# ParthaEth/GIF

Measured on AMD Instinct MI355X. Metric: G+D train-step images/sec at 256x256, batch 32/GPU, higher is better.
Workload: dtype f32

## Files before the change

### gif_amd/_lib.py

```python
import ctypes
import os

import torch

_HERE = os.path.dirname(os.path.abspath(__file__))
LIB_PATH = os.path.join(_HERE, "libgif_hip.so")

c_int, c_i64, c_float, c_void_p = ctypes.c_int, ctypes.c_int64, ctypes.c_float, ctypes.c_void_p


def knob(name, default):
    if os.environ.get("GIF_EXPERIMENTAL", "0") in ("", "0"):
        return default
    return os.environ.get(name, default)
P = c_void_p


class ConvGeom(ctypes.Structure):
    _fields_ = [(n, ctypes.c_int32) for n in ("B", "Hb", "Wb", "Cb", "Hs", "Ws", "Cs", "KH", "KW", "stride", "pad")]


class ConvEpilogue(ctypes.Structure):
    _fields_ = [("in_scale", P), ("out_scale", P), ("bias", P), ("residual", P),
                ("act", ctypes.c_int32), ("slope", c_float), ("gain", c_float),
# ... 90 lines not shown
    "gif_conv3x3_winograd_wgrad_f32": (c_int, [P, P, P, P, P, P, P, c_int, c_int, c_int, c_int, c_int, c_int, P]),
    "gif_conv3x3_winograd_wgrad_f32x3": (c_int, [P, P, P, P, P, P, P, c_int, c_int, c_int, c_int, c_int, c_int, P]),
    "gif_conv3x3_winograd_wgrad_f32h2": (c_int, [P, P, P, P, P, P, P, c_int, c_int, c_int, c_int, c_int, c_int, P]),
    "gif_winograd_unpack_wgrad_f32": (c_int, [P, P, c_int, c_int, c_int, c_int, c_int, c_i64, c_i64, c_i64, c_i64, c_float, P]),
    "gif_texture_pair_loss_partials": (c_int, [c_i64]),
    "gif_texture_pair_loss_f32": (c_int, [P, P, P, P, P, P, P, c_int, c_i64, P]),
    "gif_texture_pair_loss_bwd_f32": (c_int, [P, P, P, P, P, P, P, c_int, c_i64, P]),
    "gif_resize_f32": (c_int, [P, P, c_i64, c_int, c_int, c_int, c_int, c_int, P]),
    "gif_resize_bwd_f32": (c_int, [P, P, c_i64, c_int, c_int, c_int, c_int, c_int, P]),
    "gif_upfirdn2d_f32": (c_int, [P, P, P] + [c_int] * 13 + [EP, P]),
    "gif_bias_act_f32": (c_int, [P, P, P, P, c_i64, c_int, c_float, c_float, P]),
    "gif_colsum_partial_floats": (c_i64, [c_i64, c_int]),
    "gif_bias_act_bwd_f32": (c_int, [P, P, P, P, P, c_i64, c_int, c_float, c_float, P]),
    "gif_colsum_f32": (c_int, [P, P, P, c_i64, c_int, P]),
    "gif_mul_reduce_chunks": (c_int, [c_i64]),
    "gif_mul_reduce_f32": (c_int, [P, P, P, P, P, P, c_int, c_i64, c_int, P]),
    "gif_pack_nhwc_f32": (c_int, [P, c_int, c_int, ctypes.POINTER(c_i64), P, c_int, c_int, ctypes.POINTER(c_i64), P, c_int, c_int, c_int, c_int, P]),
    "gif_pack_nhwc_f16": (c_int, [P, c_int, c_int, ctypes.POINTER(c_i64), P, c_int, c_int, ctypes.POINTER(c_i64), P, c_int, c_int, c_int, c_int, P]),
    "gif_unpack_nhwc_f32": (c_int, [P, P, c_int, c_int, c_int, c_int, c_int, c_int, P]),
    "gif_unpack_nhwc_f16": (c_int, [P, P, c_int, c_int, c_int, c_int, c_int, c_int, P]),
    "gif_bilinear_down_f32": (c_int, [P, P, c_int, c_int, c_int, c_int, c_int, P]),
    "gif_act_inv_mul_reduce_f32": (c_int, [P, P, P, P, P, P, c_int, c_i64, c_int, c_float, c_float, P]),
    "gif_mbstd_fwd_f32": (c_int, [P, P, P, c_int, c_int, c_int, c_int, c_int, c_int, P]),
    "gif_mbstd_bwd_f32": (c_int, [P, P, P, c_int, c_int, c_int, c_int, c_int, c_int, P]),
    "gif_sqnorm_per_sample_f32": (c_int, [P, P, c_int, c_i64, P]),
    "gif_conv2d_pack_dims_f16": (c_int, [c_int, c_int, ctypes.POINTER(c_int), ctypes.POINTER(c_int)]),
    "gif_pack_weight_f16": (c_int, [P, P, c_int, c_int, c_int, c_int, c_int, c_int, c_i64, c_i64, c_i64, c_i64, c_float, P]),
    "gif_conv2d_f16_halo_eligible": (c_int, [c_int] * 7),
    "gif_conv2d_f16_halo_enable": (c_int, [c_int]),
    "gif_conv2d_fwd_f16": (c_int, [P, P, P, GP, EP, P]),
    "gif_conv2d_bwd_data_f16": (c_int, [P, P, P, GP, EP, P]),
    "gif_conv2d_wgrad_dims_f16": (c_int, [c_int, c_int, ctypes.POINTER(c_int), ctypes.POINTER(c_int)]),
    "gif_conv2d_wgrad_splits_f16": (c_int, [GP]),
    "gif_conv2d_wgrad_f16": (c_int, [P, P, P, P, P, GP, c_int, P]),
    "gif_upfirdn2d_f16": (c_int, [P, P, P] + [c_int] * 13 + [EP, P]),
    "gif_bias_act_f16": (c_int, [P, P, P, P, c_i64, c_int, c_float, c_float, P]),
    "gif_bias_act_bwd_f16": (c_int, [P, P, P, P, P, c_i64, c_int, c_float, c_float, P]),
    "gif_colsum_f16": (c_int, [P, P, P, c_i64, c_int, P]),
    "gif_mul_reduce_f16": (c_int, [P, P, P, P, P, P, c_int, c_i64, c_int, P]),
    "gif_act_inv_mul_reduce_f16": (c_int, [P, P, P, P, P, P, c_int, c_i64, c_int, c_float, c_float, P]),
    "gif_linear_nt_f32": (c_int, [P, P, P, P] + [c_int] * 7 + [c_float, c_int, c_float, c_float, P]),
    "gif_linear_nn_f32": (c_int, [P, P, P] + [c_int] * 7 + [c_float, P]),
    "gif_linear_tn_f32": (c_int, [P, P, P] + [c_int] * 6 + [c_float, P]),
    "gif_linear_bank_fwd_f32": (c_int, [P, c_int, c_int, c_int, ctypes.POINTER(LinearBankSeg), c_int, c_float, P]),
    "gif_linear_bank_bwd_f32": (c_int, [P, c_int, c_int, c_int, ctypes.POINTER(LinearBankSeg), c_int, c_float, P, c_int, c_int, P]),
    "gif_weight_sq_sum_f32": (c_int, [P, P, c_int, c_int, c_int, P]),
    "gif_style_demod_f32": (c_int, [P, P, P] + [c_int] * 7 + [c_float, c_float, P]),
    "gif_style_demod_bwd_s_f32": (c_int, [P] * 6 + [c_int] * 7 + [c_float, P]),
    "gif_style_demod_bwd_w_f32": (c_int, [P] * 4 + [c_int] * 5 + [c_float, P]),
    "gif_demod_wgrad_f32": (c_int, [P, P, P, c_int, c_int, c_int, P]),
    "gif_adam_chunk_floats": (c_int, []),
    "gif_adam_ema_step_f32": (c_int, [P, c_int, P, P, P, c_float, c_float, c_float, c_float, ctypes.c_double, ctypes.c_double,
                                      c_float, c_int, P, P, P, P]),
    "gif_prof_enable": (c_int, [c_int]),
    "gif_prof_read": (c_int, [c_int, ctypes.POINTER(ctypes.c_double), ctypes.POINTER(ctypes.c_double), ctypes.POINTER(c_i64)]),
}

_lib = None


class GifHipError(RuntimeError):
    pass


def load():
    global _lib
    if _lib is not None:
        return _lib
    if not os.path.exists(LIB_PATH):
        raise GifHipError(
            f"{LIB_PATH} not found: the HIP extension is not built. Run `make -C gif_amd/csrc` "
            "(or __graft_entry__.build()). gif_amd has no fallback path.")
    lib = ctypes.CDLL(LIB_PATH)
    for name, (res, args) in PROTOTYPES.items():
        fn = getattr(lib, name)
        fn.restype, fn.argtypes = res, args
    _lib = lib
    return lib


def check(rc, what):
    if rc != 0:
        msg = load().gif_last_error().decode(errors="replace")
        raise GifHipError(f"{what} failed (rc={rc}): {msg}")


def marshal(entry, args):
    out = list(args)
    for i, a in enumerate(out):
        if isinstance(a, torch.Tensor):
            if not a.is_contiguous():
                raise GifHipError(f"{entry}: argument {i} is not contiguous (shape {list(a.shape)}, strides {list(a.stride())})")
            out[i] = a.data_ptr()
    return out


def launch(entry, device, *args):
    fn, argv = getattr(load(), entry), marshal(entry, args)
    if device.index in (None, torch.cuda.current_device()):
        return check(fn(*argv, torch.cuda.current_stream().cuda_stream), entry)
    with torch.cuda.device(device):
        check(fn(*argv, torch.cuda.current_stream().cuda_stream), entry)


def workspace(nbytes, device):
    return torch.empty((max(nbytes // 4, 1),), device=device, dtype=torch.float32)
# ... 13 lines not shown
```

### gif_amd/functional.py

```python
import weakref

import torch
from torch.autograd import Function

from . import ops
from .ops import ConvSpec


class ActPort:
    __slots__ = ("alias", "slope", "gain", "want_bias", "parts", "y_ref")

    def __init__(self, slope, gain, want_bias):
        self.alias, self.slope, self.gain, self.want_bias = None, float(slope), float(gain), bool(want_bias)
        self.parts = []
        self.y_ref = None

    def cfg(self):
        return (self.slope, self.gain, self.want_bias, self.parts, self.y_ref)


def _observed(t):
    return t.retains_grad or bool(t._backward_hooks)


def _port_live(cfg):
    if cfg is None:
        return False
    y = cfg[4]() if cfg[4] is not None else None
    return y is None or not _observed(y)


def _file_part(parts, part):
    if not parts:
        torch.autograd.Variable._execution_engine.queue_callback(parts.clear)
    parts.append(part)


def _take_port(x, identity=False):
    port = getattr(x, "_gif_port", None)
    if (port is None or not ops.FUSE_GRAD or not torch.is_grad_enabled() or port.alias is None or not port.alias.requires_grad
            or (port.slope == 1.0 and port.gain == 1.0) != identity or _observed(x)):
        return None, None
    return port.alias, port.cfg()


_inputs_only = False


class inputs_only_backward:
    def __enter__(self):
        global _inputs_only
        self._prev, _inputs_only = _inputs_only, True

    def __exit__(self, *exc):
        global _inputs_only
        _inputs_only = self._prev
# ... 112 lines not shown
        return gs, gb, None, None, None, None, None


class ConvBiasActFn(Function):

    @staticmethod
    def forward(ctx, x, w, bias, spec, wscale, slope, gain, passthrough=False, in_port=None, parts=None, x_port=None):
        ctx.set_materialize_grads(False)
        ctx.pmask = _param_mask(x, w, bias)
        x = ops.nhwc(x)
        y, v = ops.conv_fwd(x, w, spec, wscale, keep_v=True, bias=bias, act=True, slope=slope, gain=gain)
        ctx.v = v if ctx.needs_input_grad[1] else None
        ctx.cfg = (spec, wscale, slope, gain, bias is not None)
        ctx.in_port, ctx.parts = in_port, parts
        ctx.save_for_backward(x, w, y)
        return y, y.detach(), (x.view_as(x) if passthrough else None)

    @staticmethod
    def backward(ctx, gy, g_port=None, g_alias=None):
        x, w, y = ctx.saved_tensors
        spec, ws, slope, gain, has_bias = ctx.cfg
        want_b = has_bias and _need(ctx, 2)
        gx = gw = None
        port = _port_on(ctx)
        gpre, gb = _producer_gpre(gy, g_port, y, want_b, slope, gain, ctx.parts)
        if gpre is not None:
            if ctx.needs_input_grad[0]:
                gx = _conv_dgrad(gpre, w, spec, tuple(x.shape[2:]), ws, g_alias, ctx.in_port if port else None, x)
            if _need(ctx, 1):
                gw = WgradFn.apply(gpre, x, spec, w.shape[0], w.shape[1], ws, ctx.v)
        elif ctx.needs_input_grad[0] and g_alias is not None:
            gx = _mask_into_port(ctx.in_port, g_alias, x) if port else g_alias
        return (None if port else gx), gw, (gb if want_b else None), None, None, None, None, None, None, None, (gx if port else None)


def _conv_dgrad(gpre, w, spec, big_hw, ws, residual, in_port, x):
    if in_port is None:
        return Conv2dFn.apply(gpre, w, spec, True, big_hw, ws, residual)
    slope, gain, want_b, parts = in_port[:4]
    fuse = ops.GradFuse(mask_src=x, mask_slope=slope, mask_gain=gain, want_colsum=want_b)
    gx = ops.conv_bwd_data(gpre, w, spec, big_hw, ws, residual=None if residual is None else ops.nhwc(residual), fuse=fuse)
    if want_b:
        _file_part(parts, fuse.colsum)
    return gx


def conv2d_bias_act(x, w, bias, stride=1, pad=0, wscale=1.0, slope=0.2, gain=2 ** 0.5, passthrough=False):
    x_port, in_port = _take_port(x)
    port = _new_port(True, slope, gain, bias)
    y, alias, x_alias = ConvBiasActFn.apply(x, w, bias, ConvSpec(w.shape[2], w.shape[3], stride, pad), wscale, slope, gain,
                                            bool(passthrough), in_port, None if port is None else port.parts, x_port)
    _tag(y, alias, port)
    return (y, x_alias) if passthrough else y


def conv2d(x, w, stride=1, pad=0, wscale=1.0, residual=None):
    return Conv2dFn.apply(x, w, ConvSpec(w.shape[2], w.shape[3], stride, pad), False, None, wscale, residual)


def conv_transpose2d(x, w, stride, pad, out_hw, wscale=1.0):
    return Conv2dFn.apply(x, w, ConvSpec(w.shape[2], w.shape[3], stride, pad), True, tuple(out_hw), wscale, None)


class LinearNtFn(Function):

    @staticmethod
    def forward(ctx, a, b, scale, n_pad):
        ctx.scale = scale
        ctx.pmask = _param_mask(a, b)
        ctx.save_for_backward(a, b)
        return ops.linear_nt(a, b, None, scale, n_pad=n_pad)

    @staticmethod
    def backward(ctx, g):
        a, b = ctx.saved_tensors
        N, K = b.shape
        ga = LinearNnFn.apply(g, b, ctx.scale, a.shape[1]) if _need(ctx, 0) else None
        gb = LinearTnFn.apply(g, a, ctx.scale, N, K) if _need(ctx, 1) else None
        return ga, gb, None, None


class LinearNnFn(Function):

    @staticmethod
    def forward(ctx, a, b, scale, k_pad):
        ctx.scale = scale
        ctx.pmask = _param_mask(a, b)
        ctx.save_for_backward(a, b)
        return ops.linear_nn(a, b, scale, k_pad=k_pad)

    @staticmethod
    def backward(ctx, g):
        a, b = ctx.saved_tensors
        N, K = b.shape
        ga = LinearNtFn.apply(g, b, ctx.scale, a.shape[1]) if _need(ctx, 0) else None
        gb = LinearTnFn.apply(a, g, ctx.scale, N, K) if _need(ctx, 1) else None
        return ga, gb, None, None


class LinearTnFn(Function):

    @staticmethod
    def forward(ctx, a, b, scale, N, K):
        ctx.scale = scale
        ctx.pmask = _param_mask(a, b)
        ctx.save_for_backward(a, b)
# ... 558 lines not shown
```

### gif_amd/layers.py

```python
import math
import os

import torch
from torch import nn
from torch.nn import functional as F

from . import _lib
from . import functional as GF
from .ops import cpad, pad4


_SKINNY_MAX_ROWS = int(_lib.knob("GIF_SKINNY_MAX_ROWS", "512"))


def _pad_vec(v, n):
    v = v.reshape(-1)
    k = n - v.numel()
    if k == 0:
        return v
    key = (v.device, v.dtype, k)
    tail = _ZERO_TAILS.get(key)
    if tail is None:
        tail = _ZERO_TAILS[key] = torch.zeros(k, device=v.device, dtype=v.dtype)
    return torch.cat([v, tail])
# ... 212 lines not shown
    def _padded_scales(self, style, in_act, dtype=torch.float32):
        return self.scales(style, in_act, cpad(self.out_channel, dtype))

    def forward_fused_act(self, input, style, residual, bias, slope=0.2, gain=2 ** 0.5):
        batch, in_act, height, width = input.shape
        s, d = self._padded_scales(style, in_act, input.dtype)
        w = self.weight.squeeze(0)
        if self.upsample:
            out = GF.modulated_conv2d(input, w.transpose(0, 1), s, d, stride=2, pad=0, transposed=True,
                                      out_hw=(2 * height + self.kernel_size - 2, 2 * width + self.kernel_size - 2),
                                      wscale=self.scale)
            return GF.blur_bias_act(out, self.blur.kernel, self.blur.pad, residual, bias, slope, gain)
        if self.downsample or d is None:
            return GF.bias_act(self.forward(input, style, scales=(s, d)), bias, residual, slope, gain)
        return GF.modulated_conv2d_act(input, w, s, d, residual, bias, self.padding, self.scale, slope, gain)

    def forward(self, input, style, scales=None):
        batch, in_act, height, width = input.shape
        s, d = self._padded_scales(style, in_act, input.dtype) if scales is None else scales
        w = self.weight.squeeze(0)
        if self.upsample:
            out = GF.modulated_conv2d(input, w.transpose(0, 1), s, d, stride=2, pad=0, transposed=True,
                                      out_hw=(2 * height + self.kernel_size - 2, 2 * width + self.kernel_size - 2),
                                      wscale=self.scale)
            out = self.blur(out)
        elif self.downsample:
            out = GF.modulated_conv2d(self.blur(input), w, s, d, stride=2, pad=0, wscale=self.scale)
        else:
            out = GF.modulated_conv2d(input, w, s, d, stride=1, pad=self.padding, wscale=self.scale, out_f32=self.out_fp32)
        return out


_STYLE_BANK = _lib.knob("GIF_STYLE_BANK", "1") != "0"


def modulation_bank(convs, style):
    if not _STYLE_BANK or len(convs) < 2:
        return
    x = style.reshape(-1, style.shape[-1])
    mods = [c.modulation for c in convs]
    m0 = mods[0]
    same = all(m.scale == m0.scale and m.lr_mul == 1 and m.bias is not None and m.activation is None and
               m.weight.shape[1] == m0.weight.shape[1] for m in mods)
    if not same or x.dtype != torch.float32 or x.shape[0] > _SKINNY_MAX_ROWS or any(c.in_channel > 1024 for c in convs):
        return
    weights = [m.weight for m in mods]
    if not GF.ops.linear_bank_ok(x, weights):
        return
    outs = GF.linear_bank(x, weights, [m.bias for m in mods], m0.scale)
    for c, o in zip(convs, outs):
        c._banked = (style, o)


class NoiseInjection(nn.Module):

    @staticmethod
    def small_init_weights(m):
        if hasattr(m, 'weight'):
            m.weight.data = torch.randn_like(m.weight) / 100
        if hasattr(m, 'bias'):
            m.bias.data.fill_(0.0001)

    def __init__(self, noise_in_chalnnels, noise_out_channels):
        super().__init__()
        self.noise_in_chalnnels = noise_in_chalnnels
        c = noise_in_chalnnels
        self.noise_conv = nn.Sequential(
            nn.Conv2d(c, 2 * c, 3, padding=1), nn.ReLU(),
            nn.Conv2d(2 * c, 4 * c, 3, padding=1), nn.ReLU(),
            nn.Conv2d(4 * c, noise_out_channels, 3, padding=1))
        self.noise_conv.apply(NoiseInjection.small_init_weights)

    def convolve(self, noise):
        h = noise
        for idx in (0, 2, 4):
            conv = self.noise_conv[idx]
            last = idx == 4
            h = GF.conv2d_bias_act(h, conv.weight, _pad_vec(conv.bias, cpad(conv.weight.shape[0], h.dtype)), 1, 1, 1.0,
                                   1.0 if last else 0.0, 1.0)
        return h

    def forward(self, image, noise):
        batch, _, height, width = image.shape
        if noise is None:
            noise = image.new_empty(batch, cpad(self.noise_in_chalnnels, image.dtype), height, width).normal_()
            noise[:, self.noise_in_chalnnels:] = 0
        return GF.bias_act(image, None, self.convolve(noise), 1.0, 1.0)


class ConstantInput(nn.Module):
    def __init__(self, channel, size=4):
        super().__init__()
        self.input = nn.Parameter(torch.randn(1, channel, size, size))

    def forward(self, input):
        return self.input.repeat(input.shape[0], 1, 1, 1)


class StyledConv(nn.Module):

    def __init__(self, in_channel, out_channel, kernel_size, noise_in_dims, style_dim=512, upsample=False,
                 blur_kernel=[1, 3, 3, 1], demodulate=True, apply_sqrt2_fac_in_eq_lin=False):
        super().__init__()
        self.conv = ModulatedConv2d(in_channel, out_channel, kernel_size, style_dim, upsample=upsample,
                                    blur_kernel=blur_kernel, demodulate=demodulate,
                                    apply_sqrt2_fac_in_eq_lin=apply_sqrt2_fac_in_eq_lin)
        self.noise = NoiseInjection(noise_in_dims, out_channel)
        self.activate = FusedLeakyReLU(out_channel)

    def forward(self, input, style, noise=None):
        if noise is None:
            return self.activate(self.noise(self.conv(input, style), noise=None))
        act = self.activate
        return self.conv.forward_fused_act(input, style, self.noise.convolve(noise),
                                           _pad_vec(act.bias, cpad(self.conv.out_channel, input.dtype)), act.negative_slope,
                                           act.scale)


class ToRGB(nn.Module):

    def __init__(self, in_channel, style_dim, upsample=True, blur_kernel=[1, 3, 3, 1],
                 apply_sqrt2_fac_in_eq_lin=False):
        super().__init__()
        if upsample:
            self.upsample = Upsample(blur_kernel)
        self.conv = ModulatedConv2d(in_channel, 3, 1, style_dim, demodulate=False,
                                    apply_sqrt2_fac_in_eq_lin=apply_sqrt2_fac_in_eq_lin)
        self.conv.out_fp32 = True
# ... 82 lines not shown
```

### gif_amd/ops.py

```python
import ctypes
import functools
import os
import weakref
from typing import NamedTuple, Optional

import torch

from . import _lib

CL = torch.channels_last


def _stream():
    return torch.cuda.current_stream().cuda_stream


def _device_guard(fn):
    @functools.wraps(fn)
    def wrapped(*args, **kw):
        dev = None
        for a in args + tuple(kw.values()):
            if isinstance(a, torch.Tensor) and a.is_cuda:
                if dev is None:
                    dev = a.device
# ... 549 lines not shown
    _lib.check(_fn("unpack_nhwc", g.dtype)(g.data_ptr(), out.data_ptr(), B, H, W, cp, c_off, C, _stream()), "unpack_nhwc")
    return out


def act_inv_mul_reduce(g, y, residual, bias, slope, gain):
    lib = _lib.load()
    g, y = nhwc(g), nhwc(y)
    _same_dtype(g, y, "act_inv_mul_reduce")
    B, C, H, W = y.shape
    if B * H * W == 0:
        return torch.zeros((B, C), device=y.device, dtype=torch.float32)
    nchunk = lib.gif_mul_reduce_chunks(H * W)
    out = torch.empty((B, C), device=y.device, dtype=torch.float32)
    partial = torch.empty((B * nchunk * C,), device=y.device, dtype=torch.float32)
    _lib.check(_fn("act_inv_mul_reduce", y.dtype)(g.data_ptr(), y.data_ptr(), _p(residual), _p(bias), out.data_ptr(),
                                                  partial.data_ptr(), B, H * W, C, slope, gain, _stream()),
               "act_inv_mul_reduce")
    return out


def mbstd_fwd(x, G, Cy):
    lib = _lib.load()
    x = nhwc(x)
    if x.dtype != torch.float32:
        raise _lib.GifHipError("minibatch stddev is fp32 only (functional.minibatch_stddev casts the 4x4 tensor)")
    B, C, H, W = x.shape
    y = empty_nhwc(B, Cy, H, W, x.device)
    stat = torch.empty((B // G,), device=x.device, dtype=torch.float32)
    _lib.check(lib.gif_mbstd_fwd_f32(x.data_ptr(), y.data_ptr(), stat.data_ptr(), B, H, W, C, Cy, G, _stream()), "mbstd_fwd")
    return y, stat


def mbstd_bwd(x, gy, G):
    lib = _lib.load()
    x, gy = nhwc(x), nhwc(gy)
    B, C, H, W = x.shape
    Cy = gy.shape[1]
    gx = empty_nhwc(B, C, H, W, x.device)
    _lib.check(lib.gif_mbstd_bwd_f32(x.data_ptr(), gy.data_ptr(), gx.data_ptr(), B, H, W, C, Cy, G, _stream()), "mbstd_bwd")
    return gx


def sqnorm_per_sample(g):
    lib = _lib.load()
    if not g.is_cuda or g.dtype != torch.float32:
        raise _lib.GifHipError("sqnorm_per_sample needs an fp32 device tensor")
    g = g if g.is_contiguous() or g.is_contiguous(memory_format=CL) else g.contiguous()
    B = g.shape[0]
    out = torch.empty((B,), device=g.device, dtype=torch.float32)
    _lib.check(lib.gif_sqnorm_per_sample_f32(g.data_ptr(), out.data_ptr(), B, g.numel() // max(B, 1), _stream()), "sqnorm")
    return out


_raster_ws = {}
_RASTER_WS_MAX = 8


def _raster_ws_drop(lib, key):
    ws = _raster_ws.pop(key, None)
    if ws is not None:
        lib.gif_rasterize_assume_clean_workspace(ws.data_ptr(), 0)


def _raster_workspace(lib, dev, B, F, h, w):
    key = (dev.index, torch.cuda.current_stream().cuda_stream, B, F, h, w)
    ws = _raster_ws.get(key)
    if ws is None:
        if len(_raster_ws) >= _RASTER_WS_MAX:
            _raster_ws_drop(lib, next(iter(_raster_ws)))
        ws = torch.zeros((max((lib.gif_rasterize_workspace_bytes(B, F, h, w) + 7) // 8, 1),), device=dev, dtype=torch.int64)
        _raster_ws[key] = ws
        _lib.check(lib.gif_rasterize_assume_clean_workspace(ws.data_ptr(), 1), "rasterize_assume_clean_workspace")
    return key, ws


def rasterize(face_vertices, depth, tri, out3, h, w, face_colors=None):
    lib = _lib.load()
    B, F = face_vertices.shape[:2]
    f64 = face_vertices.dtype == torch.float64
    key, ws = _raster_workspace(lib, face_vertices.device, B, F, h, w)
    plain, colors = (lib.gif_rasterize_f64, lib.gif_rasterize_colors_f64) if f64 else (lib.gif_rasterize_f32,
                                                                                        lib.gif_rasterize_colors_f32)
    if face_colors is None:
        rc = plain(face_vertices.data_ptr(), depth.data_ptr(), tri.data_ptr(), out3.data_ptr(), B, F, h, w, ws.data_ptr(),
                   _stream())
    else:
        rc = colors(face_vertices.data_ptr(), face_colors.data_ptr(), depth.data_ptr(), tri.data_ptr(), out3.data_ptr(), B, F,
                    h, w, ws.data_ptr(), _stream())
    if rc != 0:
        _raster_ws_drop(lib, key)
    _lib.check(rc, "rasterize")


def _mask_u8(m, hw):
    if m is None:
        return None
    m = m.reshape(-1)
    if m.numel() != hw:
        raise _lib.GifHipError(f"texture_pair_loss: visibility mask has {m.numel()} elements, expected {hw}")
    return (m != 0).to(torch.uint8).contiguous()


def texture_pair_loss(a, b, ma, mb, f, gloss=None):
    lib = _lib.load()
    if not (a.is_cuda and b.is_cuda and f.is_cuda) or a.dtype != torch.float32 or a.dim() != 3 or a.shape != b.shape:
        raise _lib.GifHipError("texture_pair_loss: need two fp32 device textures [C,H,W] of the same shape (no CPU fallback)")
    a, b = a.contiguous(), b.contiguous()
    C, H, W = a.shape
    HW = H * W
    f = f.to(torch.float32).reshape(-1).contiguous()
    if f.numel() != HW:
        raise _lib.GifHipError(f"texture_pair_loss: face mask has {f.numel()} elements, expected {HW}")
    ma, mb = _mask_u8(ma, HW), _mask_u8(mb, HW)
    if gloss is None:
        partial = torch.empty((lib.gif_texture_pair_loss_partials(C * HW),), device=a.device, dtype=torch.float32)
        loss = torch.empty((), device=a.device, dtype=torch.float32)
        _lib.check(lib.gif_texture_pair_loss_f32(a.data_ptr(), b.data_ptr(), _p(ma), _p(mb), f.data_ptr(), partial.data_ptr(),
                                                 loss.data_ptr(), C, HW, _stream()), "texture_pair_loss")
        return loss
    ga = torch.empty_like(a)
    gloss = gloss.to(torch.float32).contiguous()
    _lib.check(lib.gif_texture_pair_loss_bwd_f32(a.data_ptr(), b.data_ptr(), _p(ma), _p(mb), f.data_ptr(), gloss.data_ptr(),
                                                 ga.data_ptr(), C, HW, _stream()), "texture_pair_loss_bwd")
    return ga


def resize(x, out_hw, mode: str, backward_to=None):
    lib = _lib.load()
    if not x.is_cuda or x.dtype != torch.float32 or x.dim() != 4:
        raise _lib.GifHipError("resize: need a 4-D fp32 device tensor (no CPU fallback)")
    if mode not in ("bilinear", "bicubic"):
        raise _lib.GifHipError(f"resize: mode {mode!r} not supported (bilinear | bicubic)")
    x = x.contiguous()
    B, C, H, W = x.shape
    m = 0 if mode == "bilinear" else 1
    if backward_to is None:
        Ho, Wo = out_hw
        y = torch.empty((B, C, Ho, Wo), device=x.device, dtype=torch.float32)
        _lib.check(lib.gif_resize_f32(x.data_ptr(), y.data_ptr(), B * C, H, W, Ho, Wo, m, _stream()), "resize")
        return y
    Hi, Wi = backward_to
    gx = torch.empty((B, C, Hi, Wi), device=x.device, dtype=torch.float32)
    _lib.check(lib.gif_resize_bwd_f32(x.data_ptr(), gx.data_ptr(), B * C, Hi, Wi, H, W, m, _stream()), "resize_bwd")
    return gx


for _name in ("pack_weight", "conv3x3_winograd", "conv_fwd", "conv_bwd_data", "conv3x3_winograd_wgrad", "conv_wgrad", "upfirdn2d",
              "bias_act", "bias_act_bwd", "colsum", "mul_reduce", "bilinear_down", "act_inv_mul_reduce", "mbstd_fwd", "mbstd_bwd",
              "sqnorm_per_sample", "rasterize", "texture_pair_loss", "resize"):
    globals()[_name] = _device_guard(globals()[_name])
del _name


def _mat(t, what):
    if not t.is_cuda or t.dtype != torch.float32 or t.dim() != 2:
        raise _lib.GifHipError(f"{what}: need a 2-D fp32 device tensor (no CPU fallback), got {tuple(t.shape)} {t.dtype} on {t.device}")
    return t if t.stride(1) == 1 and t.stride(0) >= t.shape[1] and t.data_ptr() % 16 == 0 and t.stride(0) % 4 == 0 else t.contiguous()


def linear_nt(a, b, bias=None, scale=1.0, act=False, slope=0.2, gain=1.0, n_pad=None):
    lib = _lib.load()
    a, b = _mat(a, "linear_nt"), _mat(b, "linear_nt")
    M = a.shape[0]
    N, K = b.shape
    assert a.shape[1] >= K, (a.shape, b.shape)
    n_pad = N if n_pad is None else n_pad
    c = torch.empty((M, n_pad), device=a.device, dtype=torch.float32)
    _lib.check(lib.gif_linear_nt_f32(a.data_ptr(), b.data_ptr(), _p(bias), c.data_ptr(), M, N, K, a.stride(0), b.stride(0), n_pad,
                                     n_pad, float(scale), 1 if act else 0, float(slope), float(gain), _stream()), "linear_nt")
    return c


LINEAR_BANK_MAX = 40


def linear_bank_ok(x, weights):
    K = weights[0].shape[1]
    return (0 < len(weights) <= LINEAR_BANK_MAX and x.dtype == torch.float32 and x.dim() == 2 and x.shape[1] >= K and K % 4 == 0
            and all(w.dim() == 2 and w.shape[1] == K and w.shape[0] % 8 == 0 and w.dtype == torch.float32 for w in weights))


def _bank_segs(weights):
    segs = (_lib.LinearBankSeg * len(weights))()
    keep = []
    for g, w in zip(segs, weights):
        w = _mat(w, "linear_bank")
        assert w.stride(0) == w.shape[1], "linear_bank: weight rows must be contiguous"
        keep.append(w)
        g.w, g.n = w.data_ptr(), w.shape[0]
    return segs, keep


def linear_bank_fwd(x, weights, biases, scale):
    lib = _lib.load()
    x = _mat(x, "linear_bank_fwd")
    M, K = x.shape[0], weights[0].shape[1]
    segs, keep = _bank_segs(weights)
    outs = []
    for g, w, b in zip(segs, weights, biases):
        o = torch.empty((M, w.shape[0]), device=x.device, dtype=torch.float32)
        if b is not None:
            assert b.dtype == torch.float32 and b.numel() == w.shape[0] and b.is_contiguous()
# ... 169 lines not shown
```

### include/gif_hip.h

```cpp
#ifndef GIF_HIP_H
#define GIF_HIP_H

#include <stdint.h>

#ifdef __cplusplus
extern "C" {
#endif

#define GIF_EINVAL (-1)
#define GIF_ENOSUP (-2)

typedef void* gif_stream_t;

const char* gif_last_error(void);
int gif_abi_version(void);

int gif_f16_overflow_clear(gif_stream_t stream);
int gif_f16_overflow_or_into(float* found_inf, gif_stream_t stream);
int gif_f16_overflow_watch(int on);

#define GIF_FP32_MFMA_NATIVE 0
#define GIF_FP32_MFMA_BF16X3 1
#define GIF_FP32_MFMA_F16X2 2
int gif_set_fp32_mfma_mode(int mode);
// ... 252 lines not shown
int gif_conv2d_bwd_data_f16(const void* small, const void* wp, void* big, const gif_conv_geom* g,
                            const gif_conv_epilogue* e, gif_stream_t stream);
int gif_conv2d_wgrad_dims_f16(int Cs, int Cb, int* RP, int* CP);
int gif_conv2d_wgrad_splits_f16(const gif_conv_geom* g);
int gif_conv2d_wgrad_f16(const void* small, const void* big, float* ws, const float* small_scale, const float* big_scale,
                         const gif_conv_geom* g, int nsplit, gif_stream_t stream);
int gif_upfirdn2d_f16(const void* x, const float* k, void* y, int B, int Hi, int Wi, int C, int Ho, int Wo, int up, int down,
                      int padx0, int pady0, int KH, int KW, int flip, const gif_conv_epilogue* e, gif_stream_t stream);
int gif_bias_act_f16(const void* x, const float* bias, const void* residual, void* y, int64_t npix, int C, float slope,
                     float gain, gif_stream_t stream);
int gif_bias_act_bwd_f16(const void* gy, const void* y, void* gx, float* gbias, float* partial, int64_t npix, int C,
                         float slope, float gain, gif_stream_t stream);
int gif_colsum_f16(const void* x, float* out, float* partial, int64_t npix, int C, gif_stream_t stream);
int gif_mul_reduce_f16(const void* a, const void* b, const float* scale, void* scaled, float* out, float* partial, int B,
                       int64_t HW, int C, gif_stream_t stream);
int gif_act_inv_mul_reduce_f16(const void* g, const void* y, const void* residual, const float* bias, float* out,
                               float* partial, int B, int64_t HW, int C, float slope, float gain, gif_stream_t stream);

int gif_linear_nt_f32(const float* A, const float* B, const float* bias, float* C, int M, int N, int K, int lda, int ldb,
                      int ldc, int cpad, float scale, int act, float slope, float gain, gif_stream_t stream);
int gif_linear_nn_f32(const float* A, const float* B, float* C, int M, int N, int K, int lda, int ldb, int ldc, int cpad,
                      float scale, gif_stream_t stream);
int gif_linear_tn_f32(const float* A, const float* B, float* C, int M, int N, int K, int lda, int ldb, int ldc, float scale,
                      gif_stream_t stream);

typedef struct gif_linear_bank_seg {
    const float* w;
    const float* bias;
    float* s;
    const float* gs;
    float* gw;
    float* gbias;
    int n;
    int reserved;
} gif_linear_bank_seg;
int gif_linear_bank_fwd_f32(const float* x, int M, int K, int ldx, const gif_linear_bank_seg* segs, int nseg, float scale,
                            gif_stream_t stream);
int gif_linear_bank_bwd_f32(const float* x, int M, int K, int ldx, const gif_linear_bank_seg* segs, int nseg, float scale, float* gx,
                            int ldgx, int gx_pad, gif_stream_t stream);

typedef struct gif_adam_chunk {
    float* param;
    float* ema;
    int64_t flat_offset;
    int32_t n;
    int32_t step_offset;
} gif_adam_chunk;
int gif_adam_chunk_floats(void);
int gif_adam_ema_step_f32(const gif_adam_chunk* chunks, int nchunks, const float* grad_flat, float* exp_avg_flat,
                          float* exp_avg_sq_flat, float lr, float beta1, float beta2, float eps, double bias_correction1,
                          double bias_correction2, float ema_decay, int has_ema, const float* inv_grad_scale,
                          const float* found_inf, const float* dev_step, gif_stream_t stream);

#ifdef __cplusplus
}
#endif
#endif
```

Before: 183.7.

## Fuse first two noise-injection convs into one tiled HIP kernel with fused backward

Adds a dedicated HIP kernel that runs the first two 3x3 convs of the NoiseInjection head (6->12->24 channels, ReLU) per spatial tile. The intermediate activation stays in LDS and the convs use fp32 MFMA. A matching backward kernel fuses the ReLU masks, the data gradient through conv2 and the per-tile bias-gradient partials, then reduces them in a second small kernel. The goal is to avoid separate launches and a global-memory round trip for the small-channel intermediate, which the generic conv path handles poorly. The trade-offs are a kernel specialised to fixed channel counts, extra recompute on tile halos, and an h1 tensor still written out when gradients are needed.

```diff
diff --git a/gif_amd/_lib.py b/gif_amd/_lib.py
--- a/gif_amd/_lib.py
+++ b/gif_amd/_lib.py
@@ -166,6 +166,9 @@
     "gif_adam_chunk_floats": (c_int, []),
     "gif_adam_ema_step_f32": (c_int, [P, c_int, P, P, P, c_float, c_float, c_float, c_float, ctypes.c_double, ctypes.c_double,
                                       c_float, c_int, P, P, P, P]),
+    "gif_noise_head_partial_floats": (c_i64, [c_int, c_int, c_int]),
+    "gif_noise_head_fwd_f32": (c_int, [P] * 7 + [c_int] * 3 + [c_i64] * 8 + [c_int, P]),
+    "gif_noise_head_bwd_data_f32": (c_int, [P] * 9 + [c_int] * 3 + [c_i64] * 4 + [c_int, P]),
     "gif_prof_enable": (c_int, [c_int]),
     "gif_prof_read": (c_int, [c_int, ctypes.POINTER(ctypes.c_double), ctypes.POINTER(ctypes.c_double), ctypes.POINTER(c_i64)]),
 }
diff --git a/gif_amd/csrc/noise_head.hip b/gif_amd/csrc/noise_head.hip
--- /dev/null
+++ b/gif_amd/csrc/noise_head.hip
@@ -0,0 +1,316 @@
+#include "common.h"
+
+namespace {
+
+typedef float f32x16 __attribute__((ext_vector_type(16)));
+using gif::f32x4_t;
+
+constexpr int TH = 16, TW = 32;
+constexpr int XH = TH + 4, XW = TW + 4;
+constexpr int HH = TH + 2, HW = TW + 2;
+constexpr int C0 = 6, C0S = 8, C1 = 12, C2 = 24;
+constexpr int NT = 256;
+constexpr int K1 = C0 * 9, K1_STEPS = (K1 + 3) / 4;
+constexpr int NPOS = HH * HW, NPOS_BLOCKS = (NPOS + 15) / 16;
+constexpr int kGridCap = 512;
+constexpr int kPartialC = C2 + C1;
+
+struct WStrides {
+    long o, i, y, x;
+};
+
+struct TileGrid {
+    int tiles_y, tiles_x;
+    long ntiles;
+};
+
+__device__ __forceinline__ void tile_origin(long tile, const TileGrid& tg, int& b, int& y0, int& x0) {
+    const long per_img = (long)tg.tiles_y * tg.tiles_x;
+    b = (int)(tile / per_img);
+    const int r = (int)(tile - (long)b * per_img);
+    y0 = (r / tg.tiles_x) * TH;
+    x0 = (r % tg.tiles_x) * TW;
+}
+
+__device__ __forceinline__ float relu(float v) { return v > 0.f ? v : 0.f; }
+
+template <bool kWantH1>
+__global__ __launch_bounds__(NT, 2) void noise_head_fwd_kernel(const float* __restrict__ x, const float* __restrict__ w1, WStrides s1,
+                                                               const float* __restrict__ b1, const float* __restrict__ w2, WStrides s2,
+                                                               const float* __restrict__ b2, float* __restrict__ h1,
+                                                               float* __restrict__ h2, int H, int W, TileGrid tg) {
+    __shared__ __attribute__((aligned(16))) float sX[XH * XW * C0];
+    __shared__ __attribute__((aligned(16))) float sH[HH * HW * C1];
+    const int t = threadIdx.x, lane = t & 63, wave = t >> 6;
+    const int l16 = lane & 15, k4 = lane >> 4;
+    const int l32 = lane & 31, k2 = lane >> 5;
+
+    float w1r[K1_STEPS];
+    int xoff[K1_STEPS];
+#pragma unroll
+    for (int s = 0; s < K1_STEPS; ++s) {
+        const int k = 4 * s + k4, kc = k < K1 ? k : K1 - 1, tap = kc / C0, ci = kc % C0;
+        w1r[s] = (l16 < C1 && k < K1) ? w1[l16 * s1.o + ci * s1.i + (tap / 3) * s1.y + (tap % 3) * s1.x] : 0.f;
+        xoff[s] = ((tap / 3) * XW + tap % 3) * C0 + ci;
+    }
+    float w2r[9][C1 / 2];
+#pragma unroll
+    for (int tap = 0; tap < 9; ++tap)
+#pragma unroll
+        for (int m = 0; m < C1 / 2; ++m)
+            w2r[tap][m] = l32 < C2 ? w2[l32 * s2.o + (2 * m + k2) * s2.i + (tap / 3) * s2.y + (tap % 3) * s2.x] : 0.f;
+    f32x4_t bias1;
+#pragma unroll
+    for (int r = 0; r < 4; ++r) bias1[r] = k4 < 3 ? b1[4 * k4 + r] : 0.f;
+    f32x16 bias2;
+#pragma unroll
+    for (int r = 0; r < 16; ++r) bias2[r] = r < 12 ? b2[8 * (r / 4) + 4 * k2 + r % 4] : 0.f;
+
+    for (long tile = blockIdx.x; tile < tg.ntiles; tile += gridDim.x) {
+        int b, y0, x0;
+        tile_origin(tile, tg, b, y0, x0);
+        const size_t img = (size_t)b * H;
+
+        for (int i = t; i < XH * XW; i += NT) {
+            const int r = i / XW, c = i % XW, gy = y0 - 2 + r, gx = x0 - 2 + c;
+            float4 a = make_float4(0.f, 0.f, 0.f, 0.f);
+            float2 e = make_float2(0.f, 0.f);
+            if (gy >= 0 && gy < H && gx >= 0 && gx < W) {
+                const float* p = x + ((img + gy) * W + gx) * C0S;
+                a = *reinterpret_cast<const float4*>(p);
+                e = *reinterpret_cast<const float2*>(p + 4);
+            }
+            float2* d = reinterpret_cast<float2*>(sX + i * C0);
+            d[0] = make_float2(a.x, a.y);
+            d[1] = make_float2(a.z, a.w);
+            d[2] = e;
+        }
+        __syncthreads();
+
+        for (int blk = wave; blk < NPOS_BLOCKS; blk += NT / 64) {
+            const int pos = blk * 16 + l16, pc = pos < NPOS ? pos : NPOS - 1;
+            const float* xp = sX + ((pc / HW) * XW + pc % HW) * C0;
+            f32x4_t acc = bias1;
+#pragma unroll
+            for (int s = 0; s < K1_STEPS; ++s) acc = __builtin_amdgcn_mfma_f32_16x16x4f32(w1r[s], xp[xoff[s]], acc, 0, 0, 0);
+            const int r = pos / HW, c = pos % HW, gy = y0 - 1 + r, gx = x0 - 1 + c;
+            if (pos < NPOS && k4 < 3) {
+                const bool inside = gy >= 0 && gy < H && gx >= 0 && gx < W;
+                f32x4_t v;
+#pragma unroll
+                for (int q = 0; q < 4; ++q) v[q] = inside ? relu(acc[q]) : 0.f;
+                float* d = sH + pos * C1;
+                *reinterpret_cast<float2*>(d + 2 * k4) = make_float2(v[0], v[2]);
+                *reinterpret_cast<float2*>(d + 6 + 2 * k4) = make_float2(v[1], v[3]);
+                if (kWantH1 && inside && r >= 1 && r <= TH && c >= 1 && c <= TW)
+                    *reinterpret_cast<f32x4_t*>(h1 + ((img + gy) * W + gx) * C1 + 4 * k4) = v;
+            }
+        }
+        __syncthreads();
+
+        {
+            f32x16 acc[4];
+#pragma unroll
+            for (int p = 0; p < 4; ++p) acc[p] = bias2;
+#pragma unroll
+            for (int tap = 0; tap < 9; ++tap)
+#pragma unroll
+                for (int p = 0; p < 4; ++p) {
+                    const float2* s =
+                        reinterpret_cast<const float2*>(sH + ((wave * 4 + p + tap / 3) * HW + l32 + tap % 3) * C1 + k2 * (C1 / 2));
+                    const float2 v0 = s[0], v1 = s[1], v2 = s[2];
+                    const float hv[C1 / 2] = {v0.x, v0.y, v1.x, v1.y, v2.x, v2.y};
+#pragma unroll
+                    for (int m = 0; m < C1 / 2; ++m) acc[p] = __builtin_amdgcn_mfma_f32_32x32x2f32(w2r[tap][m], hv[m], acc[p], 0, 0, 0);
+                }
+            const int gx = x0 + l32;
+#pragma unroll
+            for (int p = 0; p < 4; ++p) {
+                const int gy = y0 + wave * 4 + p;
+                if (gy < H && gx < W) {
+                    float* g = h2 + ((img + gy) * W + gx) * C2 + 4 * k2;
+#pragma unroll
+                    for (int q = 0; q < 3; ++q) {
+                        f32x4_t v;
+#pragma unroll
+                        for (int r = 0; r < 4; ++r) v[r] = relu(acc[p][4 * q + r]);
+                        *reinterpret_cast<f32x4_t*>(g + 8 * q) = v;
+                    }
+                }
+            }
+        }
+    }
+}
+
+constexpr int GQ = C2 / 4;
+constexpr int GROW = HW * GQ;
+__global__ __launch_bounds__(NT, 2) void noise_head_bwd_kernel(const float* __restrict__ g2, const float* __restrict__ h2,
+                                                               const float* __restrict__ h1, const float* __restrict__ w2, WStrides s2,
+                                                               float* __restrict__ gp2, float* __restrict__ gp1,
+                                                               float* __restrict__ partial, int H, int W, TileGrid tg) {
+    __shared__ __attribute__((aligned(16))) float sG[HH * GQ * HW * 4];
+    __shared__ float sRed[(NT / 64) * C1];
+    const int t = threadIdx.x, lane = t & 63, wave = t >> 6;
+    const int l16 = lane & 15, k4 = lane >> 4;
+    float wr[9][GQ];
+#pragma unroll
+    for (int tap = 0; tap < 9; ++tap)
+#pragma unroll
+        for (int q = 0; q < GQ; ++q)
+            wr[tap][q] = l16 < C1 ? w2[(4 * q + k4) * s2.o + l16 * s2.i + (tap / 3) * s2.y + (tap % 3) * s2.x] : 0.f;
+
+    for (long tile = blockIdx.x; tile < tg.ntiles; tile += gridDim.x) {
+        int b, y0, x0;
+        tile_origin(tile, tg, b, y0, x0);
+        const size_t img = (size_t)b * H;
+        __syncthreads();
+        for (int i = t; i < HH * GROW; i += NT) {
+            const int r = i / GROW, f = i % GROW, cc = f / GQ, q = f % GQ, gy = y0 - 1 + r, gx = x0 - 1 + cc;
+            float4 v = make_float4(0.f, 0.f, 0.f, 0.f);
+            if (gy >= 0 && gy < H && gx >= 0 && gx < W) {
+                const size_t off = ((img + gy) * W + gx) * C2 + 4 * q;
+                const float4 g = *reinterpret_cast<const float4*>(g2 + off);
+                const float4 a = *reinterpret_cast<const float4*>(h2 + off);
+                v = make_float4(a.x > 0.f ? g.x : 0.f, a.y > 0.f ? g.y : 0.f, a.z > 0.f ? g.z : 0.f, a.w > 0.f ? g.w : 0.f);
+                if (r >= 1 && r <= TH && cc >= 1 && cc <= TW) *reinterpret_cast<float4*>(gp2 + off) = v;
+            }
+            *reinterpret_cast<float4*>(sG + ((r * GQ + q) * HW + cc) * 4) = v;
+        }
+        __syncthreads();
+
+        {
+            const int ch = t >> 3, sub = t & 7;
+            float s = 0.f;
+            if (ch < C2)
+                for (int k = 0; k < TH * TW / 8; ++k) {
+                    const int i = sub + 8 * k;
+                    s += sG[(((i / TW + 1) * GQ + ch / 4) * HW + (i % TW) + 1) * 4 + ch % 4];
+                }
+#pragma unroll
+            for (int m = 1; m < 8; m <<= 1) s += __shfl_xor(s, m);
+            if (ch < C2 && sub == 0) partial[tile * kPartialC + ch] = s;
+        }
+
+        f32x4_t acc[4][2];
+#pragma unroll
+        for (int p = 0; p < 4; ++p)
+#pragma unroll
+            for (int hf = 0; hf < 2; ++hf) acc[p][hf] = (f32x4_t)(0.f);
+#pragma unroll
+        for (int tap = 0; tap < 9; ++tap)
+#pragma unroll
+            for (int p = 0; p < 4; ++p)
+#pragma unroll
+                for (int hf = 0; hf < 2; ++hf) {
+                    const float* s = sG + ((wave * 4 + p + 2 - tap / 3) * GQ * HW + 16 * hf + l16 + 2 - tap % 3) * 4 + k4;
+#pragma unroll
+                    for (int q = 0; q < GQ; ++q)
+                        acc[p][hf] = __builtin_amdgcn_mfma_f32_16x16x4f32(wr[tap][q], s[q * HW * 4], acc[p][hf], 0, 0, 0);
+                }
+
+        f32x4_t s = (f32x4_t)(0.f);
+#pragma unroll
+        for (int p = 0; p < 4; ++p)
+#pragma unroll
+            for (int hf = 0; hf < 2; ++hf) {
+                const int gy = y0 + wave * 4 + p, gx = x0 + 16 * hf + l16;
+                if (k4 < 3 && gy < H && gx < W) {
+                    const size_t off = ((img + gy) * W + gx) * C1 + 4 * k4;
+                    const f32x4_t a = *reinterpret_cast<const f32x4_t*>(h1 + off);
+                    f32x4_t v;
+#pragma unroll
+                    for (int r = 0; r < 4; ++r) v[r] = a[r] > 0.f ? acc[p][hf][r] : 0.f;
+                    *reinterpret_cast<f32x4_t*>(gp1 + off) = v;
+                    s += v;
+                }
+            }
+#pragma unroll
+        for (int r = 0; r < 4; ++r) {
+            float v = s[r];
+#pragma unroll
+            for (int m = 1; m < 16; m <<= 1) v += __shfl_xor(v, m);
+            s[r] = v;
+        }
+        if (l16 == 0 && k4 < 3)
+#pragma unroll
+            for (int r = 0; r < 4; ++r) sRed[wave * C1 + 4 * k4 + r] = s[r];
+        __syncthreads();
+        if (t < C1) {
+            float v = sRed[t];
+#pragma unroll
+            for (int wv = 1; wv < NT / 64; ++wv) v += sRed[wv * C1 + t];
+            partial[tile * kPartialC + C2 + t] = v;
+        }
+    }
+}
+
+__global__ __launch_bounds__(256) void noise_head_reduce_kernel(const float* __restrict__ partial, long rows, float* __restrict__ gb2,
+                                                                float* __restrict__ gb1) {
+    __shared__ float sm[256];
+    const int c = blockIdx.x, t = threadIdx.x;
+    float s = 0.f;
+    for (long r = t; r < rows; r += 256) s += partial[r * kPartialC + c];
+    sm[t] = s;
+    __syncthreads();
+    for (int m = 128; m > 0; m >>= 1) {
+        if (t < m) sm[t] += sm[t + m];
+        __syncthreads();
+    }
+    if (t == 0) (c < C2 ? gb2[c] : gb1[c - C2]) = sm[0];
+}
+
+void tile_grid(int B, int H, int W, TileGrid& tg) {
+    tg.tiles_y = (H + TH - 1) / TH;
+    tg.tiles_x = (W + TW - 1) / TW;
+    tg.ntiles = (long)B * tg.tiles_y * tg.tiles_x;
+}
+
+int launch_blocks(long ntiles, int grid_cap) {
+    const long cap = grid_cap > 0 ? grid_cap : kGridCap;
+    return (int)(ntiles < cap ? ntiles : cap);
+}
+
+}
+
+extern "C" {
+
+int64_t gif_noise_head_partial_floats(int B, int H, int W) {
+    if (B <= 0 || H <= 0 || W <= 0) return 0;
+    TileGrid tg;
+    tile_grid(B, H, W, tg);
+    return tg.ntiles * kPartialC;
+}
+
+int gif_noise_head_fwd_f32(const float* x, const float* w1, const float* b1, const float* w2, const float* b2, float* h1, float* h2,
+                           int B, int H, int W, int64_t w1_so, int64_t w1_si, int64_t w1_sy, int64_t w1_sx, int64_t w2_so,
+                           int64_t w2_si, int64_t w2_sy, int64_t w2_sx, int grid_cap, gif_stream_t stream) {
+    GIF_REQUIRE(B >= 0 && H >= 0 && W >= 0, "noise_head_fwd: bad dims (B=%d H=%d W=%d)", B, H, W);
+    if (B == 0 || H == 0 || W == 0) return 0;
+    GIF_REQUIRE(x && w1 && b1 && w2 && b2 && h2, "noise_head_fwd: null pointer");
+    TileGrid tg;
+    tile_grid(B, H, W, tg);
+    const WStrides s1{w1_so, w1_si, w1_sy, w1_sx}, s2{w2_so, w2_si, w2_sy, w2_sx};
+    hipStream_t s = gif::as_stream(stream);
+    const int grid = launch_blocks(tg.ntiles, grid_cap);
+    if (h1)
+        noise_head_fwd_kernel<true><<<grid, NT, 0, s>>>(x, w1, s1, b1, w2, s2, b2, h1, h2, H, W, tg);
+    else
+        noise_head_fwd_kernel<false><<<grid, NT, 0, s>>>(x, w1, s1, b1, w2, s2, b2, nullptr, h2, H, W, tg);
+    return gif::check_launch("noise_head_fwd");
+}
+
+int gif_noise_head_bwd_data_f32(const float* g2, const float* h2, const float* h1, const float* w2, float* gp2, float* gp1, float* gb2,
+                                float* gb1, float* partial, int B, int H, int W, int64_t w2_so, int64_t w2_si, int64_t w2_sy,
+                                int64_t w2_sx, int grid_cap, gif_stream_t stream) {
+    GIF_REQUIRE(B > 0 && H > 0 && W > 0, "noise_head_bwd_data: bad dims (B=%d H=%d W=%d)", B, H, W);
+    GIF_REQUIRE(g2 && h2 && h1 && w2 && gp2 && gp1 && gb2 && gb1 && partial, "noise_head_bwd_data: null pointer");
+    TileGrid tg;
+    tile_grid(B, H, W, tg);
+    const WStrides s2{w2_so, w2_si, w2_sy, w2_sx};
+    hipStream_t s = gif::as_stream(stream);
+    noise_head_bwd_kernel<<<launch_blocks(tg.ntiles, grid_cap), NT, 0, s>>>(g2, h2, h1, w2, s2, gp2, gp1, partial, H, W, tg);
+    noise_head_reduce_kernel<<<kPartialC, 256, 0, s>>>(partial, tg.ntiles, gb2, gb1);
+    return gif::check_launch("noise_head_bwd_data");
+}
+
+}
diff --git a/gif_amd/functional.py b/gif_amd/functional.py
--- a/gif_amd/functional.py
+++ b/gif_amd/functional.py
@@ -2,6 +2,7 @@
 
 import torch
 from torch.autograd import Function
+from torch.autograd.function import once_differentiable
 
 from . import ops
 from .ops import ConvSpec
@@ -220,6 +221,35 @@
                                             bool(passthrough), in_port, None if port is None else port.parts, x_port)
     _tag(y, alias, port)
     return (y, x_alias) if passthrough else y
+
+
+class NoiseHeadFn(Function):
+
+    @staticmethod
+    def forward(ctx, x, w1, b1, w2, b2, grad):
+        if ctx.needs_input_grad[0]:
+            raise ops._lib.GifHipError("noise_head has no gradient w.r.t. its input: use the three-conv path (NoiseInjection.convolve does)")
+        ctx.pmask = _param_mask(x, w1, b1, w2, b2)
+        x = ops.nhwc(x)
+        h1, h2 = ops.noise_head_fwd(x, w1, b1, w2, b2, want_h1=grad)
+        if grad:
+            ctx.save_for_backward(x, w1, w2, h1, h2)
+        return h2
+
+    @staticmethod
+    @once_differentiable
+    def backward(ctx, g2):
+        x, w1, w2, h1, h2 = ctx.saved_tensors
+        gp2, gp1, gb2, gb1 = ops.noise_head_bwd_data(g2, h2, h1, w2)
+        spec = ConvSpec(3, 3, 1, 1)
+        gw1 = ops.conv_wgrad(gp1, x, spec, w1.shape[0], w1.shape[1]) if _need(ctx, 1) else None
+        gw2 = ops.conv_wgrad(gp2, h1, spec, w2.shape[0], w2.shape[1]) if _need(ctx, 3) else None
+        return None, gw1, (gb1 if _need(ctx, 2) else None), gw2, (gb2 if _need(ctx, 4) else None), None
+
+
+def noise_head(x, w1, b1, w2, b2):
+    grad = torch.is_grad_enabled() and any(t.requires_grad for t in (w1, b1, w2, b2))
+    return NoiseHeadFn.apply(x, w1, b1, w2, b2, grad)
 
 
 def conv2d(x, w, stride=1, pad=0, wscale=1.0, residual=None):
diff --git a/gif_amd/layers.py b/gif_amd/layers.py
--- a/gif_amd/layers.py
+++ b/gif_amd/layers.py
@@ -288,6 +288,9 @@
         c._banked = (style, o)
 
 
+_NOISE_HEAD = _lib.knob("GIF_NOISE_HEAD", "1") != "0"
+
+
 class NoiseInjection(nn.Module):
 
     @staticmethod
@@ -307,9 +310,17 @@
             nn.Conv2d(4 * c, noise_out_channels, 3, padding=1))
         self.noise_conv.apply(NoiseInjection.small_init_weights)
 
+    def _fused_head(self, noise):
+        c0, c1 = self.noise_conv[0], self.noise_conv[2]
+        return (_NOISE_HEAD and not noise.requires_grad and c0.bias is not None and c1.bias is not None
+                and c0.bias.is_cuda and c1.bias.is_cuda and GF.ops.noise_head_ok(noise, c0.weight, c1.weight))
+
     def convolve(self, noise):
-        h = noise
-        for idx in (0, 2, 4):
+        h, rest = noise, (0, 2, 4)
+        if self._fused_head(noise):
+            c0, c1 = self.noise_conv[0], self.noise_conv[2]
+            h, rest = GF.noise_head(noise, c0.weight, c0.bias, c1.weight, c1.bias), (4,)
+        for idx in rest:
             conv = self.noise_conv[idx]
             last = idx == 4
             h = GF.conv2d_bias_act(h, conv.weight, _pad_vec(conv.bias, cpad(conv.weight.shape[0], h.dtype)), 1, 1, 1.0,
diff --git a/gif_amd/ops.py b/gif_amd/ops.py
--- a/gif_amd/ops.py
+++ b/gif_amd/ops.py
@@ -625,6 +625,56 @@
     return out
 
 
+NOISE_HEAD_CHANNELS = (6, 12, 24)
+
+
+def noise_head_ok(x, w1, w2):
+    c0, c1, c2 = NOISE_HEAD_CHANNELS
+    return (x.is_cuda and w1.is_cuda and w2.is_cuda and x.dtype == w1.dtype == w2.dtype == torch.float32 and x.dim() == 4
+            and x.shape[1] == pad4(c0) and tuple(w1.shape) == (c1, c0, 3, 3) and tuple(w2.shape) == (c2, c1, 3, 3))
+
+
+def _noise_head_vec(b, n, what):
+    if b.dtype != torch.float32 or tuple(b.shape) != (n,):
+        raise _lib.GifHipError(f"noise_head: {what} must be an fp32 vector of {n}, got {tuple(b.shape)} {b.dtype}")
+    return b.contiguous()
+
+
+def noise_head_fwd(x, w1, b1, w2, b2, want_h1=False, grid_cap=0):
+    if not noise_head_ok(x, w1, w2):
+        raise _lib.GifHipError(f"noise_head_fwd: unsupported operands (x {tuple(x.shape)} {x.dtype}, w1 {tuple(w1.shape)}, w2 {tuple(w2.shape)})")
+    x = nhwc(x)
+    B, _, H, W = x.shape
+    c0, c1, c2 = NOISE_HEAD_CHANNELS
+    b1, b2 = _noise_head_vec(b1, c1, "b1"), _noise_head_vec(b2, c2, "b2")
+    h1 = empty_nhwc(B, c1, H, W, x.device) if want_h1 else None
+    h2 = empty_nhwc(B, c2, H, W, x.device)
+    _lib.check(_lib.load().gif_noise_head_fwd_f32(x.data_ptr(), w1.data_ptr(), b1.data_ptr(), w2.data_ptr(), b2.data_ptr(), _p(h1),
+                                                  h2.data_ptr(), B, H, W, *w1.stride(), *w2.stride(), int(grid_cap), _stream()),
+               "noise_head_fwd")
+    return h1, h2
+
+
+def noise_head_bwd_data(g2, h2, h1, w2, grid_cap=0):
+    lib = _lib.load()
+    g2, h2, h1 = nhwc(g2), nhwc(h2), nhwc(h1)
+    B, c2, H, W = h2.shape
+    c1 = h1.shape[1]
+    if ((c1, c2) != NOISE_HEAD_CHANNELS[1:] or g2.shape != h2.shape or tuple(h1.shape) != (B, c1, H, W) or tuple(w2.shape) != (c2, c1, 3, 3)
+            or not g2.dtype == h2.dtype == h1.dtype == w2.dtype == torch.float32):
+        raise _lib.GifHipError(f"noise_head_bwd_data: unsupported operands (g2 {tuple(g2.shape)}, h2 {tuple(h2.shape)}, h1 {tuple(h1.shape)})")
+    dev = h2.device
+    gp2, gp1 = empty_nhwc(B, c2, H, W, dev), empty_nhwc(B, c1, H, W, dev)
+    if B * H * W == 0:
+        return gp2, gp1, torch.zeros((c2,), device=dev), torch.zeros((c1,), device=dev)
+    gb2, gb1 = torch.empty((c2,), device=dev), torch.empty((c1,), device=dev)
+    partial = torch.empty((lib.gif_noise_head_partial_floats(B, H, W),), device=dev)
+    _lib.check(lib.gif_noise_head_bwd_data_f32(g2.data_ptr(), h2.data_ptr(), h1.data_ptr(), w2.data_ptr(), gp2.data_ptr(), gp1.data_ptr(),
+                                               gb2.data_ptr(), gb1.data_ptr(), partial.data_ptr(), B, H, W, *w2.stride(), int(grid_cap),
+                                               _stream()), "noise_head_bwd_data")
+    return gp2, gp1, gb2, gb1
+
+
 _raster_ws = {}
 _RASTER_WS_MAX = 8
 
@@ -720,7 +770,7 @@
 
 for _name in ("pack_weight", "conv3x3_winograd", "conv_fwd", "conv_bwd_data", "conv3x3_winograd_wgrad", "conv_wgrad", "upfirdn2d",
               "bias_act", "bias_act_bwd", "colsum", "mul_reduce", "bilinear_down", "act_inv_mul_reduce", "mbstd_fwd", "mbstd_bwd",
-              "sqnorm_per_sample", "rasterize", "texture_pair_loss", "resize"):
+              "sqnorm_per_sample", "noise_head_fwd", "noise_head_bwd_data", "rasterize", "texture_pair_loss", "resize"):
     globals()[_name] = _device_guard(globals()[_name])
 del _name
 
diff --git a/include/gif_hip.h b/include/gif_hip.h
--- a/include/gif_hip.h
+++ b/include/gif_hip.h
@@ -328,6 +328,14 @@
                           double bias_correction2, float ema_decay, int has_ema, const float* inv_grad_scale,
                           const float* found_inf, const float* dev_step, gif_stream_t stream);
 
+int64_t gif_noise_head_partial_floats(int B, int H, int W);
+int gif_noise_head_fwd_f32(const float* x, const float* w1, const float* b1, const float* w2, const float* b2, float* h1, float* h2,
+                           int B, int H, int W, int64_t w1_so, int64_t w1_si, int64_t w1_sy, int64_t w1_sx, int64_t w2_so,
+                           int64_t w2_si, int64_t w2_sy, int64_t w2_sx, int grid_cap, gif_stream_t stream);
+int gif_noise_head_bwd_data_f32(const float* g2, const float* h2, const float* h1, const float* w2, float* gp2, float* gp1, float* gb2,
+                                float* gb1, float* partial, int B, int H, int W, int64_t w2_so, int64_t w2_si, int64_t w2_sy,
+                                int64_t w2_sx, int grid_cap, gif_stream_t stream);
+
 #ifdef __cplusplus
 }
 #endif
```

Measured after the change: 185.2, median of 6. Within noise of the previous version (+0.8%).
